# dayne-2stacks/Fingerprint-Matching-Code

Hardware: AMD Instinct MI355X
Metric: graph-match pairs/sec @ n=256 kpts, batch=1024, 1 & 8 GPU (higher is better)
Workload: dtype bf16

## Files before the change

fingerprint-matching-code_amd/csrc/gemm.hip:

```cpp
#include "gemm_phase.h"
#include "gemm_pp.h"
#include <cstdlib>
#include <cstring>

namespace fpm {
int& gemm_bn256_min();
}

extern "C" int fpm_gemm(int dtype, const void* A, long lda, long sA, const int* a_rows, const void* B, long ldb,
                        long sB, int M, int N, int K, int batch, int epi, const float* bias, float* Cf, void* Ct,
                        long ldc, long sC, const int* n1, const int* n2, void* stream) {
    using namespace fpm;
    FPM_CHECK_ARG(dtype == 0 || dtype == 1, "gemm: dtype must be 0 (f32) or 1 (bf16)");
    FPM_CHECK_ARG(M >= 0 && N > 0 && K > 0 && batch >= 0, "gemm: bad sizes M=%d N=%d K=%d", M, N, K);
    FPM_CHECK_ARG(K % (dtype ? 8 : 4) == 0, "gemm: K=%d must be a multiple of %d", K, dtype ? 8 : 4);
    FPM_CHECK_ARG(lda % (dtype ? 8 : 4) == 0 && ldb % (dtype ? 8 : 4) == 0, "gemm: lda/ldb must keep rows 16-B aligned");
    FPM_CHECK_ARG((epi != EPI_AFFINITY && epi != EPI_HALF_AFFINITY) || (n1 && n2),
                  "gemm: affinity epilogues need n1/n2");
    FPM_CHECK_ARG(epi >= EPI_STORE && epi <= EPI_HALF_AFFINITY, "gemm: bad epilogue %d", epi);
    if (M == 0 || batch == 0) return 0;
    GemmParams p = {};
    p.A = A; p.lda = lda; p.sA = sA; p.a_rows = a_rows;
    p.B = B; p.ldb = ldb; p.sB = sB; p.sB_seg = 0;
    p.row_scale = nullptr;
    p.M = M; p.N = N; p.K = K; p.nseg = 1;
    p.tile_info = nullptr; p.group_off = nullptr;
    p.epi = epi; p.bias = bias; p.Cf = Cf; p.Ct = Ct; p.ldc = ldc; p.sC = sC; p.n1 = n1; p.n2 = n2;
    hipStream_t st = (hipStream_t)stream;
    const int mt = (M + G2_BM - 1) / G2_BM;
    const bool epi_ok = epi == EPI_STORE || epi == EPI_RELU || (epi == EPI_AFFINITY && Cf && !Ct);
    const bool big = dtype == 1 && M >= G2_BM && K % G2_BK == 0 && N % 8 == 0 && lda % 8 == 0 && ldb % 8 == 0 &&
                     !(Cf && Ct) && (Cf ? ldc % 4 == 0 : ldc % 8 == 0) && epi_ok &&
                     (long)mt * ((N + 127) / 128) * batch >= 128;
    if (big) {
        const int BN = (N % 256 == 0 && (long)mt * (N / 256) * batch >= gemm_bn256_min()) ? 256 : 128;
        p.remap_mtiles = mt;
        dim3 grid(remap_grid_big(N, BN, mt), 1, batch);
        const bool f32 = Cf != nullptr;
        const bool phase = BN == 256 && use_gemm_phase(K);
#define FPM_BIG(BN_, E_, F_)                                                                            \
    do {                                                                                               \
        if (BN_ == 256 && phase) hipLaunchKernelGGL((gemm_phase_kernel<E_, F_>), grid, dim3(G2_THREADS), 0, st, p); \
        else hipLaunchKernelGGL((gemm_big_kernel<BN_, E_, F_>), grid, dim3(G2_THREADS), 0, st, p);      \
    } while (0)
        if (epi == EPI_AFFINITY) {
            if (BN == 256) FPM_BIG(256, EPI_AFFINITY, true); else FPM_BIG(128, EPI_AFFINITY, true);
        } else if (BN == 256) {
            if (epi == EPI_RELU) { if (f32) FPM_BIG(256, EPI_RELU, true); else FPM_BIG(256, EPI_RELU, false); }
            else { if (f32) FPM_BIG(256, EPI_STORE, true); else FPM_BIG(256, EPI_STORE, false); }
        } else {
            if (epi == EPI_RELU) { if (f32) FPM_BIG(128, EPI_RELU, true); else FPM_BIG(128, EPI_RELU, false); }
            else { if (f32) FPM_BIG(128, EPI_STORE, true); else FPM_BIG(128, EPI_STORE, false); }
        }
#undef FPM_BIG
        return check_launch("fpm_gemm");
    }
    p.remap_mtiles = (M + GBM - 1) / GBM;
    dim3 grid(remap_grid(N, p.remap_mtiles), 1, batch);
    if (dtype == 0) hipLaunchKernelGGL((gemm_kernel<float, false>), grid, dim3(GTHREADS), 0, st, p);
    else hipLaunchKernelGGL((gemm_kernel<bf16_t, false>), grid, dim3(GTHREADS), 0, st, p);
    return check_launch("fpm_gemm");
}

namespace fpm {
int& gemm_pp_flag() {
    static int on = [] {
        const char* e = getenv("FPM_GEMM_PP");
        return e ? atoi(e) : 0;
    }();
    return on;
}

int& gemm_phase_flag() {
    static int on = [] {
        const char* e = getenv("FPM_GEMM_PHASE");
        return e ? atoi(e) : 1;
    }();
    return on;
}

int& gemm_bn256_min() {
    static int v = [] {
        const char* e = getenv("FPM_GEMM_BN256_MIN");
        return e ? atoi(e) : 512;
    }();
    return v;
}
}

extern "C" int fpm_gemm_norm_max(const void* A, long lda, const void* B, long ldb, int M, int N, int K,
                                 const float* bias, const float* res, long ldres, const float* nw, const float* nb,
                                 float eps, int P, float* gmax, void* stream) {
    using namespace fpm;
    FPM_CHECK_ARG(P == G2_BM || 2 * P == G2_BM, "gemm_norm_max: P=%d must be %d or %d (one or two pairs per tile)", P,
                  G2_BM, G2_BM / 2);
    FPM_CHECK_ARG(M >= 0 && M % P == 0 && N > 0 && K > 0 && K % G2_BK == 0, "gemm_norm_max: bad sizes M=%d N=%d K=%d",
                  M, N, K);
    FPM_CHECK_ARG(lda % 8 == 0 && ldb % 8 == 0 && ldres >= N, "gemm_norm_max: bad strides");
    FPM_CHECK_ARG(res && nw && nb && gmax, "gemm_norm_max: null operand");
    if (M == 0) return 0;
    GemmParams p = {};
    p.A = A; p.lda = lda; p.B = B; p.ldb = ldb;
    p.M = M; p.N = N; p.K = K; p.nseg = 1;
    p.epi = EPI_NORM_MAX; p.bias = bias; p.ldc = ldres;
    p.res = res; p.nw = nw; p.nb = nb; p.eps = eps; p.gmax = gmax; p.norm_p = P;
    const int mt = (M + G2_BM - 1) / G2_BM;
    p.remap_mtiles = mt;
    dim3 grid(remap_grid_big(N, 128, mt), 1, 1);
    hipLaunchKernelGGL((gemm_big_kernel<128, EPI_NORM_MAX, true>), grid, dim3(G2_THREADS), 0, (hipStream_t)stream, p);
    return fpm::check_launch("fpm_gemm_norm_max");
}
// ... 77 lines not shown
    float* X1c = ws + (long)B * d;
    if (fpm_gemm(0, w, kw, 0, nullptr, A_w, kw, 0, B, d, kw, 1, EPI_TANH, A_b, coef, nullptr, d, 0, nullptr, nullptr,
                 stream))
        return 1;
    hipLaunchKernelGGL(rows_scale_kernel, dim3((unsigned)((long)B * n1max)), dim3(256), 0, (hipStream_t)stream, X1,
                       ld1, n1max, d, coef, X1c);
    if (check_launch("fpm_affinity_fwd")) return 1;
    return fpm_gemm(0, X1c, d, (long)n1max * d, nullptr, X2, ld2, (long)n2max * ld2, n1max, n2max, d, B,
                    epi == 0 ? EPI_AFFINITY : EPI_HALF_AFFINITY, nullptr, K, nullptr, ldk, (long)n1max * ldk, n2, n1,
                    stream);
}

int& plan_graph_flag();
int& combine_npb_flag();
int& sinkhorn_bwd_reg_flag();
int& sinkhorn_fast_flag();
int& sinkhorn_lform_flag();
int& soft_topk_fast_flag();
int& afau_attn_v_flag();
int& gnn_store_sc1_flag();
int& combine_store_sc1_flag();
int& gemm_store_sc1_flag();
int& combine_lds_kb_flag();
int& gnn_mlp_off_flag();
int& outer_sum_vec_flag();
int& gnn_sweeps_flag();
int& scatter_f32_rows_flag();
int& scatter_batch_flag();
int& afau_head_split_flag();

extern "C" int fpm_set_tuning(const char* key, int value) {
    int* f = nullptr;
    if (key && !strcmp(key, "gemm_phase")) f = &fpm::gemm_phase_flag();
    else if (key && !strcmp(key, "gemm_pp")) f = &fpm::gemm_pp_flag();
    else if (key && !strcmp(key, "plan_graph")) f = &plan_graph_flag();
    else if (key && !strcmp(key, "combine_npb")) f = &combine_npb_flag();
    else if (key && !strcmp(key, "sinkhorn_bwd_reg")) f = &sinkhorn_bwd_reg_flag();
    else if (key && !strcmp(key, "sinkhorn_fast")) f = &sinkhorn_fast_flag();
    else if (key && !strcmp(key, "sinkhorn_lform")) f = &sinkhorn_lform_flag();
    else if (key && !strcmp(key, "topk_fast")) f = &soft_topk_fast_flag();
    else if (key && !strcmp(key, "afau_attn_v")) f = &afau_attn_v_flag();
    else if (key && !strcmp(key, "gnn_store_sc1")) f = &gnn_store_sc1_flag();
    else if (key && !strcmp(key, "combine_store_sc1")) f = &combine_store_sc1_flag();
    else if (key && !strcmp(key, "gemm_store_sc1")) f = &gemm_store_sc1_flag();
    else if (key && !strcmp(key, "combine_lds_kb")) f = &combine_lds_kb_flag();
    else if (key && !strcmp(key, "gnn_mlp_off")) f = &gnn_mlp_off_flag();
    else if (key && !strcmp(key, "outer_sum_vec")) f = &outer_sum_vec_flag();
    else if (key && !strcmp(key, "gnn_sweeps")) f = &gnn_sweeps_flag();
    else if (key && !strcmp(key, "scatter_f32_rows")) f = &scatter_f32_rows_flag();
    else if (key && !strcmp(key, "scatter_batch")) f = &scatter_batch_flag();
    else if (key && !strcmp(key, "afau_head_split")) f = &afau_head_split_flag();
    if (!f) {
        fpm::set_error("fpm_set_tuning: unknown key '%s'", key ? key : "(null)");
        return -1;
    }
    if (f == &gnn_mlp_off_flag() && value != 0) {
        const char* e = getenv("FPM_TIMING_PROBES");
        if (!e || strcmp(e, "1") != 0) {
            fpm::set_error("fpm_set_tuning: '%s' is a timing probe with wrong results; set FPM_TIMING_PROBES=1 "
                           "to allow it", key);
            return -1;
        }
    }
    const int prev = *f;
    *f = value;
    return prev;
}
// ... 156 lines not shown
```

fingerprint-matching-code_amd/csrc/gemm_core.h:

```cpp
#pragma once
#include "fpm_common.h"

namespace fpm {

enum GemmEpi : int {
    EPI_STORE = 0,
    EPI_RELU = 1,
    EPI_TANH = 2,
    EPI_AFFINITY = 3,
    EPI_HALF_AFFINITY = 4,
    EPI_NORM_MAX = 5,
    EPI_NORM_OUT = 6,
};

struct GemmParams {
    const void* A;
    long lda, sA;
    const int* a_rows;
    const void* B;
    long ldb, sB, sB_seg;
    const float* row_scale;
    int M, N, K, nseg;
    const int* tile_info;
    const int* group_off;
    int epi;
    const float* bias;
    float* Cf;
    void* Ct;
    long ldc, sC;
    const int* n1;
    const int* n2;
    int remap_mtiles;
    const float* res;
    const float* nw;
    const float* nb;
    float eps;
    float* gmax;
    long ldt;
    int split;
    int norm_p;
    int store_sc1;
    int remap_cm;
};

constexpr int REMAP_MIN = 32;
inline unsigned remap_grid(int N, int mtiles) {
    long nt = (N + 127) / 128, chunk = 4 * nt;
    long t = nt * mtiles;
    if (mtiles < REMAP_MIN) return (unsigned)t;
    return (unsigned)((t + 8 * chunk - 1) / (8 * chunk) * (8 * chunk));
}
__device__ __forceinline__ int remap_tile(int nt, int mtiles, int cm = 4) {
    if (mtiles < REMAP_MIN) return blockIdx.x;
    const int chunk = cm * nt;
    const int i = blockIdx.x >> 3;
    return ((i / chunk) * 8 + (blockIdx.x & 7)) * chunk + (i % chunk);
}

typedef __bf16 bf16x8_t __attribute__((ext_vector_type(8)));
typedef float f32x4_t __attribute__((ext_vector_type(4)));

template <typename T> struct TileCfg;
template <> struct TileCfg<float> {
    static constexpr int BK = 32;
    static constexpr int EPC = 4;
};
template <> struct TileCfg<bf16_t> {
    static constexpr int BK = 64;
    static constexpr int EPC = 8;
};

constexpr int GBM = 128, GBN = 128, GTHREADS = 256;
constexpr int LDS_ROW_BYTES = 144;
constexpr int LDS_TILE_BYTES = GBM * LDS_ROW_BYTES;

// ... 197 lines not shown
```

fingerprint-matching-code_amd/csrc/gemm_phase.h:

```cpp
#pragma once
#include <type_traits>
#include "gemm_big.h"

namespace fpm {

constexpr int GP_HALF = 128 * 128;
constexpr int GP_SMEM = g2_max(8 * GP_HALF, G2_BM * (2 * 256 + 16));
constexpr int GP_MIN_KTILES = 2;

#define FPM_VMCNT(N) asm volatile("s_waitcnt vmcnt(" #N ")" ::: "memory")

#ifdef GP_PROBE
__device__ unsigned long long* gp_probe_buf;
#define GP_STAMP(k)                                                                                   \
    do {                                                                                              \
        const unsigned long long t_ = __builtin_amdgcn_s_memtime();                                   \
        if (threadIdx.x == 0 && gp_probe_buf)                                                         \
            gp_probe_buf[((long)blockIdx.z * gridDim.x + blockIdx.x) * 8 + (k)] = t_;                   \
    } while (0)
#else
#define GP_STAMP(k)
#endif

#ifndef GP_STAGGER
// ... 263 lines not shown
                for (int fm = 0; fm < 4; ++fm)
#pragma unroll
                    for (int j = 0; j < 4; ++j) {
                        const int r = wr * 64 + fm * 16 + (lane >> 4) * 4 + j;
#pragma unroll
                        for (int fn = 0; fn < 2; ++fn) {
                            const int c = g * 128 + wc * 32 + fn * 16 + (lane & 15);
                            const int n = n0 + c < p.N ? n0 + c : p.N - 1;
                            *(float*)(smem + r * ROW + c * 4) =
                                g2_epi<EPI, HB>(p.bias, acc[h][g][fm][fn][j], row0 + h * 128 + r, n, n1b, n2b);
                        }
                    }
        };
#pragma unroll
        for (int h = 0; h < 2; ++h) {
            if (p.bias) image(h, std::true_type{});
            else image(h, std::false_type{});
            __syncthreads();
#pragma unroll 4
            for (int it = 0; it < 128 * CH / G2_THREADS; ++it) {
                const int idx = it * G2_THREADS + tid;
                const int r = idx / CH, ch = idx % CH;
                const int gr = row0 + h * 128 + r;
                if (gr < row_end && n0 + ch * 4 < p.N) {
                    uint4 v = *(const uint4*)(smem + r * ROW + ch * 16);
                    *(uint4*)(Cf + (long)gr * p.ldc + n0 + ch * 4) = v;
                }
            }
            __syncthreads();
        }
    }
}

#undef FPM_VMCNT

int& gemm_phase_flag();
inline bool use_gemm_phase(int K) { return gemm_phase_flag() != 0 && K / G2_BK >= GP_MIN_KTILES; }

}
```

fingerprint-matching-code_amd/csrc/gemm_pp.h:

```cpp
#pragma once
#include <type_traits>
#include "gemm_big.h"

namespace fpm {

constexpr int PP_BM = 256, PP_BN = 128, PP_BK = 32, PP_THREADS = 256, PP_NST = 3;
constexpr int PP_A_BYTES = PP_BM * PP_BK * 2;
constexpr int PP_B_BYTES = PP_BN * PP_BK * 2;
constexpr int PP_STAGE = PP_A_BYTES + PP_B_BYTES;
constexpr int PP_ROW_OUT = PP_BN * 2 + 16;
constexpr int PP_SMEM = g2_max(PP_NST * PP_STAGE, PP_BM * PP_ROW_OUT);
static_assert(PP_SMEM <= 80 * 1024, "two workgroups per CU need <= 80 KB of LDS each");

inline unsigned pp_grid(int N, int mtiles) { return remap_grid_big(N, PP_BN, mtiles); }

__device__ __forceinline__ int pp_slot(int chunk, int row) {
    return ((0x2130 >> (4 * chunk)) & 3) ^ ((row >> 2) & 3);
}
__device__ __forceinline__ int pp_chunk(int slot, int row) {
    return (0x1320 >> (4 * (slot ^ ((row >> 2) & 3)))) & 3;
}

template <int EPI>
__global__ __launch_bounds__(PP_THREADS, 2) void gemm_pp_kernel(GemmParams p) {
    __shared__ __attribute__((aligned(16))) unsigned char smem[PP_SMEM];
    const int tid = threadIdx.x, lane = tid & 63, wave = tid >> 6;
    const int wr = wave >> 1, wc = wave & 1;
    const int batch = blockIdx.z;

    const int nt = (p.N + PP_BN - 1) / PP_BN;
    const int q = remap_tile(nt, p.remap_mtiles);
    const int mtile = q / nt, ntile = q - mtile * nt;
    if (mtile >= p.remap_mtiles) return;
    int group = 0, row0, row_end;
    if (p.tile_info) {
        group = p.tile_info[2 * mtile];
        if (group < 0) return;
        row0 = p.tile_info[2 * mtile + 1];
        row_end = p.group_off[group + 1];
    } else {
        row0 = mtile * PP_BM;
        row_end = p.M;
    }
    const int n0 = ntile * PP_BN;
    const bf16_t* A = (const bf16_t*)p.A + (long)batch * p.sA;
    const bf16_t* Bg = (const bf16_t*)p.B + (long)batch * p.sB + (long)group * p.sB_seg;

    const bf16_t* asrc[4];
    const bf16_t* bsrc[2];
#pragma unroll
    for (int i = 0; i < 4; ++i) {
        const int r = (wave * 4 + i) * 16 + (lane >> 2);
        int gr = row0 + r;
        gr = gr < row_end ? gr : row0;
        const long arow = p.a_rows ? (long)p.a_rows[gr] : (long)gr;
        asrc[i] = A + arow * p.lda + pp_chunk(lane & 3, r) * 8;
    }
#pragma unroll
    for (int i = 0; i < 2; ++i) {
        const int r = (wave * 2 + i) * 16 + (lane >> 2);
        const int n = n0 + r < p.N ? n0 + r : p.N - 1;
        bsrc[i] = Bg + (long)n * p.ldb + pp_chunk(lane & 3, r) * 8;
    }
    auto issue = [&](int stage, int kt) {
        unsigned char* As = smem + stage * PP_STAGE;
        unsigned char* Bs = As + PP_A_BYTES;
        const int k0 = kt * PP_BK;
#pragma unroll
        for (int i = 0; i < 4; ++i)
            __builtin_amdgcn_global_load_lds((gbl_ptr_t)(asrc[i] + k0), (lds_ptr_t)(As + (wave * 4 + i) * 1024), 16,
                                             0, 0);
#pragma unroll
        for (int i = 0; i < 2; ++i)
            __builtin_amdgcn_global_load_lds((gbl_ptr_t)(bsrc[i] + k0), (lds_ptr_t)(Bs + (wave * 2 + i) * 1024), 16,
                                             0, 0);
    };

    const int so = pp_slot(lane >> 4, lane & 15) * 16;
    const int a_off = (wr * 64 + (lane & 15)) * 64 + so;
    const int b_off = (wc * 64 + (lane & 15)) * 64 + so;

    f32x4_t acc[2][4][4];
#pragma unroll
    for (int h = 0; h < 2; ++h)
#pragma unroll
        for (int i = 0; i < 4; ++i)
#pragma unroll
            for (int j = 0; j < 4; ++j) acc[h][i][j] = f32x4_t{0.f, 0.f, 0.f, 0.f};

    auto compute = [&](int stage) __attribute__((always_inline)) {
        const unsigned char* As = smem + stage * PP_STAGE;
        const unsigned char* Bs = As + PP_A_BYTES;
        bf16x8_t a[2][4], b[4];
#pragma unroll
        for (int f = 0; f < 4; ++f) b[f] = *(const bf16x8_t*)(Bs + b_off + f * 1024);
#pragma unroll
        for (int h = 0; h < 2; ++h)
#pragma unroll
            for (int f = 0; f < 4; ++f) a[h][f] = *(const bf16x8_t*)(As + a_off + h * 8192 + f * 1024);
#pragma unroll
        for (int h = 0; h < 2; ++h)
#pragma unroll
            for (int fm = 0; fm < 4; ++fm)
#pragma unroll
                for (int fn = 0; fn < 4; ++fn)
                    acc[h][fm][fn] = __builtin_amdgcn_mfma_f32_16x16x32_bf16(a[h][fm], b[fn], acc[h][fm][fn], 0, 0, 0);
    };

    const int ktiles = p.K / PP_BK;
    issue(0, 0);
    if (ktiles > 1) issue(1, 1);
    for (int kt = 0; kt < ktiles; ++kt) {
        if (kt + 1 < ktiles) asm volatile("s_waitcnt vmcnt(6)" ::: "memory");
        else asm volatile("s_waitcnt vmcnt(0)" ::: "memory");
        __builtin_amdgcn_s_barrier();
        if (kt + 2 < ktiles) issue((kt + 2) % PP_NST, kt + 2);
        compute(kt % PP_NST);
    }
    __syncthreads();

    int n1b = 0, n2b = 0;
    if (EPI == EPI_AFFINITY) { n1b = p.n1[batch]; n2b = p.n2[batch]; }
    constexpr int ROW = PP_ROW_OUT;
    const int lr = wr * 64 + (lane >> 4) * 4, lc = wc * 64 + (lane & 15);
    auto image = [&](auto hb) __attribute__((always_inline)) {
        constexpr bool HB = decltype(hb)::value;
#pragma unroll
        for (int h = 0; h < 2; ++h) {
            int wo = (h * 128 + lr) * ROW + lc * 2;
            asm volatile("" : "+v"(wo));
            unsigned char* wb = smem + wo;
#pragma unroll
            for (int fm = 0; fm < 4; ++fm)
#pragma unroll
                for (int j = 0; j < 4; j += 2) {
                    const int r = h * 128 + lr + fm * 16 + j;
#pragma unroll
                    for (int fn = 0; fn < 4; ++fn) {
                        const int c = lc + fn * 16;
                        const int n = n0 + c < p.N ? n0 + c : p.N - 1;
                        const uint32_t pk =
                            f2bf2(g2_epi<EPI, HB>(p.bias, acc[h][fm][fn][j], row0 + r, n, n1b, n2b),
                                  g2_epi<EPI, HB>(p.bias, acc[h][fm][fn][j + 1], row0 + r + 1, n, n1b, n2b));
                        const int off = (fm * 16 + j) * ROW + fn * 32;
                        *(bf16_t*)(wb + off) = (bf16_t)pk;
                        *(bf16_t*)(wb + off + ROW) = (bf16_t)(pk >> 16);
                    }
                }
        }
    };
    if (p.bias) image(std::true_type{});
    else image(std::false_type{});
    __syncthreads();
    bf16_t* Ct = (bf16_t*)p.Ct + (long)batch * p.sC;
    constexpr int CH = PP_BN / 8;
    if (p.store_sc1) {
        typedef unsigned int u32x4_t __attribute__((ext_vector_type(4)));
        const __amdgpu_buffer_rsrc_t rc = __builtin_amdgcn_make_buffer_rsrc(
            (void*)(Ct + (long)row0 * p.ldc + n0), (short)0, (int)(PP_BM * p.ldc * 2), 0x00020000);
#pragma unroll 4
        for (int it = 0; it < PP_BM * CH / PP_THREADS; ++it) {
            const int idx = it * PP_THREADS + tid;
            const int r = idx / CH, ch = idx % CH;
            if (row0 + r < row_end && n0 + ch * 8 < p.N) {
                const uint4 v = *(const uint4*)(smem + r * ROW + ch * 16);
                const u32x4_t pk = {v.x, v.y, v.z, v.w};
                __builtin_amdgcn_raw_buffer_store_b128(pk, rc, (int)((r * p.ldc + ch * 8) * 2), 0, 16);
            }
        }
    } else {
#pragma unroll 4
        for (int it = 0; it < PP_BM * CH / PP_THREADS; ++it) {
            const int idx = it * PP_THREADS + tid;
            const int r = idx / CH, ch = idx % CH;
            if (row0 + r < row_end && n0 + ch * 8 < p.N) {
                const uint4 v = *(const uint4*)(smem + r * ROW + ch * 16);
                *(uint4*)(Ct + (long)(row0 + r) * p.ldc + n0 + ch * 8) = v;
            }
        }
    }
}

int& gemm_pp_flag();
inline bool use_gemm_pp(int K) { return gemm_pp_flag() != 0 && K % 64 == 0 && K >= PP_BK; }

}
```

fingerprint-matching-code_amd/csrc/spline.hip:

```cpp
#include "gemm_phase.h"
#include "gemm_pp.h"

#include <vector>

namespace {

struct ProfRec {
    hipEvent_t a, b;
    int slot;
};
bool g_prof_on = false;
std::vector<ProfRec> g_prof;
int* g_prof_rows = nullptr;
constexpr int PROF_MAX = 4096;

constexpr int NCELL = 26;

struct PlanLayout {
    long mask, indeg, dslot, basis_e, grp_e, blk_cnt, cell_off, rowid, arows, tile_info, tile_info2, dst_ptr, csr_e,
        nbr_local, rows4, basis4, total;
    long nblk, max_rows, max_tiles, max_tiles2;
};

__host__ __device__ inline long al(long x) { return (x + 255) & ~255L; }

__host__ __device__ inline long plan_max_rows(long E, long num_nodes) {
    long a = 4 * E, b = 25 * num_nodes;
    return (a < b ? a : b) + num_nodes;
}

__host__ __device__ PlanLayout plan_layout(long E, long num_nodes) {
    PlanLayout L;
    L.nblk = (num_nodes + 255) / 256;
    L.max_rows = plan_max_rows(E, num_nodes);
// ... 1093 lines not shown
                                   void* stream) {
    return fpm_spline_conv_fwd_argmax(dtype, x_op, plan_ws, E, num_nodes, nmax, nvalid, W, bias, y_ws, y_ws_bytes, mode,
                                      xres, cscale, out_f, out_t, nullptr, stream);
}

extern "C" int fpm_spline_conv_fwd_argmax(int dtype, const void* x_op, const void* plan_ws, long E, long num_nodes,
                                          int nmax, const int* nvalid, const void* W, const float* bias, void* y_ws,
                                          long y_ws_bytes, int mode, const float* xres, const float* cscale,
                                          float* out_f, void* out_t, int* argmax, void* stream) {
    using namespace fpm;
    FPM_CHECK_ARG(dtype == 0 || dtype == 1, "spline_conv: bad dtype");
    FPM_CHECK_ARG(mode >= 0 && mode <= 5 && (!(mode & 1) || xres), "spline_conv: mode %d: bit 0 (residual) needs xres, "
                  "mode >> 1 must be 0, 1 or 2", mode);
    FPM_CHECK_ARG(!(mode >> 1) || (dtype == 1 && out_t && !argmax),
                  "spline_conv: split operand rows (mode >> 1) need bf16 out_t (inference forward)");
    FPM_CHECK_ARG(y_ws_bytes >= fpm_spline_y_bytes(dtype, E, num_nodes), "spline_conv: y workspace too small");
    PlanLayout L = plan_layout(E, num_nodes);
    const char* w = (const char*)plan_ws;
    hipStream_t st = (hipStream_t)stream;
    const int D = 768;
    {
        GemmParams p = {};
        p.A = x_op; p.lda = D; p.a_rows = (const int*)(w + L.arows);
        p.B = W; p.ldb = D; p.sB_seg = (long)D * D;
        p.M = (int)L.max_rows; p.N = D; p.K = D; p.nseg = 1;
        p.tile_info = (const int*)(w + L.tile_info);
        p.group_off = (const int*)(w + L.cell_off);
        p.epi = EPI_STORE; p.ldc = D;
        if (dtype == 0) p.Cf = (float*)y_ws;
        else p.Ct = y_ws;
        p.store_sc1 = gemm_store_sc1_flag();
        p.remap_mtiles = (int)(dtype == 0 ? L.max_tiles : L.max_tiles2);
        if (dtype == 1) p.tile_info = (const int*)(w + L.tile_info2);
        const bool pp = dtype == 1 && use_gemm_pp(D);
        dim3 grid(dtype == 0 ? remap_grid(D, p.remap_mtiles) : pp ? pp_grid(D, p.remap_mtiles)
                                                                  : remap_grid256(D, p.remap_mtiles), 1, 1);
        ProfRec rec = {nullptr, nullptr, (int)g_prof.size()};
        if (g_prof_on && !g_prof_rows) (void)hipMalloc(&g_prof_rows, PROF_MAX * sizeof(int));
        if (g_prof_on && g_prof_rows && rec.slot < PROF_MAX) {
            (void)hipMemcpyAsync(g_prof_rows + rec.slot, w + L.cell_off + NCELL * sizeof(int), sizeof(int),
                                 hipMemcpyDeviceToDevice, st);
            (void)hipEventCreate(&rec.a);
            (void)hipEventCreate(&rec.b);
            (void)hipEventRecord(rec.a, st);
        }
        if (dtype == 0) hipLaunchKernelGGL((gemm_kernel<float, false>), grid, dim3(GTHREADS), 0, st, p);
        else if (pp) hipLaunchKernelGGL((gemm_pp_kernel<EPI_STORE>), grid, dim3(PP_THREADS), 0, st, p);
        else if (use_gemm_phase(D)) hipLaunchKernelGGL((gemm_phase_kernel<EPI_STORE, false>), grid, dim3(G2_THREADS), 0, st, p);
        else hipLaunchKernelGGL((gemm_big_kernel<256, EPI_STORE, false>), grid, dim3(G2_THREADS), 0, st, p);
        if (g_prof_on && g_prof_rows && rec.slot < PROF_MAX) {
            (void)hipEventRecord(rec.b, st);
            g_prof.push_back(rec);
        }
    }
    {
        const long graphs = (num_nodes + nmax - 1) / nmax;
        const int npb = combine_npb_flag();
#define FPM_COMB(T_, N_)                                                                                         \
    do {                                                                                                         \
        const dim3 cg((unsigned)(((graphs + 7) / 8) * 8 * ((nmax + N_ - 1) / N_)));                              \
        const size_t lds = (size_t)combine_lds_kb_flag() * 1024;                                                 \
        if (combine_store_sc1_flag() && !(mode >> 1))                                                            \
            hipLaunchKernelGGL((combine_kernel<T_, N_, false, 16>), cg, dim3(64 * N_), lds, st, (const T_*)y_ws, \
                               (const int*)(w + L.cell_off), bias, (const int*)(w + L.dst_ptr),                 \
                               (const int4*)(w + L.rows4), (const float4*)(w + L.basis4), num_nodes, nmax,       \
                               nvalid, mode, xres, cscale, out_f, (T_*)out_t, nullptr);                          \
        else                                                                                                     \
            hipLaunchKernelGGL((combine_kernel<T_, N_>), cg, dim3(64 * N_), lds, st, (const T_*)y_ws,            \
                               (const int*)(w + L.cell_off), bias, (const int*)(w + L.dst_ptr),                 \
                               (const int4*)(w + L.rows4), (const float4*)(w + L.basis4), num_nodes, nmax,       \
                               nvalid, mode, xres, cscale, out_f, (T_*)out_t, nullptr);                          \
    } while (0)
        if (argmax) {
#define FPM_COMBA(T_)                                                                                            \
    hipLaunchKernelGGL((combine_kernel<T_, 4, true>), dim3((unsigned)(((graphs + 7) / 8) * 8 * ((nmax + 3) / 4))), \
                       dim3(256), 0, st, (const T_*)y_ws, (const int*)(w + L.cell_off), bias,                    \
                       (const int*)(w + L.dst_ptr), (const int4*)(w + L.rows4), (const float4*)(w + L.basis4),   \
                       num_nodes, nmax, nvalid, mode, xres, cscale, out_f, (T_*)out_t, argmax)
            if (dtype == 0) FPM_COMBA(float); else FPM_COMBA(bf16_t);
#undef FPM_COMBA
// ... 374 lines not shown
```

Before: 32220.

## Add strip-walking bf16 GEMM kernel that processes two M-tiles per workgroup

New measurement: 32760, median of 6. 1.7% higher.

```diff
diff --git a/fingerprint-matching-code_amd/csrc/gemm.hip b/fingerprint-matching-code_amd/csrc/gemm.hip
--- a/fingerprint-matching-code_amd/csrc/gemm.hip
+++ b/fingerprint-matching-code_amd/csrc/gemm.hip
@@ -1,11 +1,11 @@
 #include "gemm_phase.h"
-#include "gemm_pp.h"
 #include <cstdlib>
 #include <cstring>
 
 namespace fpm {
 int& gemm_bn256_min();
 }
+int& gemm_store_sc1_flag();
 
 extern "C" int fpm_gemm(int dtype, const void* A, long lda, long sA, const int* a_rows, const void* B, long ldb,
                         long sB, int M, int N, int K, int batch, int epi, const float* bias, float* Cf, void* Ct,
@@ -47,7 +47,13 @@
             if (BN == 256) FPM_BIG(256, EPI_AFFINITY, true); else FPM_BIG(128, EPI_AFFINITY, true);
         } else if (BN == 256) {
             if (epi == EPI_RELU) { if (f32) FPM_BIG(256, EPI_RELU, true); else FPM_BIG(256, EPI_RELU, false); }
-            else { if (f32) FPM_BIG(256, EPI_STORE, true); else FPM_BIG(256, EPI_STORE, false); }
+            else if (f32) FPM_BIG(256, EPI_STORE, true);
+            else {
+                const int S = phase ? gemm_walk_strip(p) : 0;
+                p.store_sc1 = gemm_store_sc1_flag();
+                if (S != 0) gemm_walk_launch(p, S, batch, st);
+                else FPM_BIG(256, EPI_STORE, false);
+            }
         } else {
             if (epi == EPI_RELU) { if (f32) FPM_BIG(128, EPI_RELU, true); else FPM_BIG(128, EPI_RELU, false); }
             else { if (f32) FPM_BIG(128, EPI_STORE, true); else FPM_BIG(128, EPI_STORE, false); }
@@ -63,20 +69,31 @@
 }
 
 namespace fpm {
-int& gemm_pp_flag() {
-    static int on = [] {
-        const char* e = getenv("FPM_GEMM_PP");
-        return e ? atoi(e) : 0;
-    }();
-    return on;
-}
-
 int& gemm_phase_flag() {
     static int on = [] {
         const char* e = getenv("FPM_GEMM_PHASE");
         return e ? atoi(e) : 1;
     }();
     return on;
+}
+
+int& gemm_walk_flag() {
+    static int v = [] {
+        const char* e = getenv("FPM_GEMM_WALK");
+        return e ? atoi(e) : GW_AUTO;
+    }();
+    return v;
+}
+
+int gemm_cu_count() {
+    static int cus = [] {
+        int dev = 0, n = 0;
+        if (hipGetDevice(&dev) != hipSuccess ||
+            hipDeviceGetAttribute(&n, hipDeviceAttributeMultiprocessorCount, dev) != hipSuccess || n <= 0)
+            n = 256;
+        return n;
+    }();
+    return cus;
 }
 
 int& gemm_bn256_min() {
@@ -220,7 +237,8 @@
 extern "C" int fpm_set_tuning(const char* key, int value) {
     int* f = nullptr;
     if (key && !strcmp(key, "gemm_phase")) f = &fpm::gemm_phase_flag();
-    else if (key && !strcmp(key, "gemm_pp")) f = &fpm::gemm_pp_flag();
+    else if (key && !strcmp(key, "gemm_walk")) f = &fpm::gemm_walk_flag();
+    else if (key && !strcmp(key, "gemm_bn256_min")) f = &fpm::gemm_bn256_min();
     else if (key && !strcmp(key, "plan_graph")) f = &plan_graph_flag();
     else if (key && !strcmp(key, "combine_npb")) f = &combine_npb_flag();
     else if (key && !strcmp(key, "sinkhorn_bwd_reg")) f = &sinkhorn_bwd_reg_flag();
diff --git a/fingerprint-matching-code_amd/csrc/gemm_core.h b/fingerprint-matching-code_amd/csrc/gemm_core.h
--- a/fingerprint-matching-code_amd/csrc/gemm_core.h
+++ b/fingerprint-matching-code_amd/csrc/gemm_core.h
@@ -41,6 +41,9 @@
     int norm_p;
     int store_sc1;
     int remap_cm;
+    int walk;
+    const int* tile_count;
+    int walk_cus;
 };
 
 constexpr int REMAP_MIN = 32;
diff --git a/fingerprint-matching-code_amd/csrc/gemm_phase.h b/fingerprint-matching-code_amd/csrc/gemm_phase.h
--- a/fingerprint-matching-code_amd/csrc/gemm_phase.h
+++ b/fingerprint-matching-code_amd/csrc/gemm_phase.h
@@ -319,9 +319,334 @@
     }
 }
 
+constexpr int GW_SMEM = 8 * GP_HALF;
+constexpr int GW_MAX_S = 2;
+
+__host__ __device__ inline int gemm_walk_rule(int tiles, int wgs, int cus) {
+    const long r1 = ((long)tiles * wgs + cus - 1) / cus, r2 = ((long)((tiles + 1) / 2) * wgs + cus - 1) / cus;
+    return 2 * r2 * 7 <= r1 * 8 ? 2 : 1;
+}
+
+#ifdef GP_PROBE
+#define GW_STAMP(k) do { if (ti == 0) GP_STAMP(k); } while (0)
+#else
+#define GW_STAMP(k)
+#endif
+
+template <bool SC1>
+__global__ __launch_bounds__(G2_THREADS, 1) void gemm_walk_kernel(GemmParams p) {
+    constexpr int BN = 256;
+    __shared__ __attribute__((aligned(16))) unsigned char smem[GW_SMEM];
+    const int tid = threadIdx.x, lane = tid & 63, wave = tid >> 6;
+    const int wr = wave >> 2, wc = wave & 3;
+    const int batch = blockIdx.z;
+
+    const int nt = p.N / BN;
+    int mtiles = p.remap_mtiles;
+    if (p.tile_count) mtiles = *p.tile_count < mtiles ? *p.tile_count : mtiles;
+    const int S = p.walk > 0 ? p.walk : gemm_walk_rule(mtiles, nt * (int)gridDim.z, p.walk_cus);
+    const int strips = (mtiles + S - 1) / S;
+    const int i = blockIdx.x >> 3;
+    const int strip = (i / nt) * 8 + (blockIdx.x & 7), ntile = i % nt;
+    if (strip >= strips) return;
+    int t_row0[GW_MAX_S], t_rend[GW_MAX_S], t_grp[GW_MAX_S];
+    unsigned ok = 0;
+#pragma unroll
+    for (int j = 0; j < GW_MAX_S; ++j) {
+        const int mt = strip * S + j;
+        t_row0[j] = 0; t_rend[j] = 0; t_grp[j] = 0;
+        if (j < S && mt < mtiles) {
+            if (p.tile_info) {
+                const int g = p.tile_info[2 * mt];
+                if (g >= 0) {
+                    t_grp[j] = g;
+                    t_row0[j] = p.tile_info[2 * mt + 1];
+                    t_rend[j] = p.group_off[g + 1];
+                    ok |= 1u << j;
+                }
+            } else {
+                t_row0[j] = mt * G2_BM;
+                t_rend[j] = p.M;
+                ok |= 1u << j;
+            }
+        }
+    }
+    if (!ok) return;
+    constexpr int m_end = GW_MAX_S;
+    auto next_valid = [&](int j) __attribute__((always_inline)) {
+        const unsigned r = j < GW_MAX_S ? ok >> j : 0u;
+        return r ? j + __builtin_ctz(r) : GW_MAX_S;
+    };
+    auto pick = [&](const int (&t)[GW_MAX_S], int j) __attribute__((always_inline)) {
+        return j == 0 ? t[0] : t[1];
+    };
+    int m = next_valid(0);
+
+    const int n0 = ntile * BN;
+    const bf16_t* A = (const bf16_t*)p.A + (long)batch * p.sA;
+    const unsigned char* Bb = (const unsigned char*)((const bf16_t*)p.B + (long)batch * p.sB);
+    bf16_t* Ct = (bf16_t*)p.Ct + (long)batch * p.sC;
+
+    auto tile_at = [&](int j, int& row0, int& row_end, const unsigned char*& bg) __attribute__((always_inline)) {
+        row0 = pick(t_row0, j);
+        row_end = pick(t_rend, j);
+        bg = Bb + (long)pick(t_grp, j) * p.sB_seg * 2;
+    };
+    auto a_rows_of = [&](int row0, int row_end, int (&ar)[2][2]) __attribute__((always_inline)) {
+#pragma unroll
+        for (int i = 0; i < 2; ++i)
+#pragma unroll
+            for (int h = 0; h < 2; ++h) {
+                int gr = row0 + h * 128 + (wave * 2 + i) * 8 + (lane >> 3);
+                gr = gr < row_end ? gr : row0;
+                ar[h][i] = p.a_rows ? p.a_rows[gr] : gr;
+            }
+    };
+    const uint32_t kc16 = (uint32_t)(((lane & 7) ^ (lane >> 4)) * 16);
+    uint32_t b_off[2];
+#pragma unroll
+    for (int i = 0; i < 2; ++i)
+        b_off[i] = (uint32_t)((n0 + (wave * 2 + i) * 8 + (lane >> 3)) * (uint32_t)p.ldb * 2) + (kc16 ^ (i * 64));
+    const uint32_t lda2 = (uint32_t)p.lda * 2, bhalf = 128 * (uint32_t)p.ldb * 2;
+    const unsigned char* Ab = (const unsigned char*)A;
+
+    int row0, row_end, row0n = 0, row_endn = 0;
+    const unsigned char *bg, *bgn = nullptr;
+    int ar[2][2], arn[2][2];
+
+    auto issue = [&](int slot, int buf, const int (&rows)[2][2], const unsigned char* bgrp, int k0) __attribute__((always_inline)) {
+        unsigned char* dst = smem + (buf * 4 + slot) * GP_HALF + wave * 2048;
+        if (slot < 2) {
+            const unsigned char* ab = Ab + 2 * k0;
+#pragma unroll
+            for (int i = 0; i < 2; ++i)
+                __builtin_amdgcn_global_load_lds(
+                    (gbl_ptr_t)(ab + ((uint64_t)(uint32_t)rows[slot][i] * lda2 + (kc16 ^ (i * 64)))),
+                    (lds_ptr_t)(dst + i * 1024), 16, 0, 0);
+        } else {
+            const unsigned char* b = bgrp + 2 * k0 + (slot - 2) * bhalf;
+            __builtin_amdgcn_global_load_lds((gbl_ptr_t)(b + b_off[0]), (lds_ptr_t)dst, 16, 0, 0);
+            __builtin_amdgcn_global_load_lds((gbl_ptr_t)(b + b_off[1]), (lds_ptr_t)(dst + 1024), 16, 0, 0);
+        }
+    };
+
+    const int xr = (lane >> 1) & 7;
+    const int a_off = (wr * 64 + (lane & 15)) * 128;
+    const int b_offl = (wc * 32 + (lane & 15)) * 128;
+    const int s0 = ((lane >> 4) ^ xr) * 16, s1 = ((4 + (lane >> 4)) ^ xr) * 16;
+
+    f32x4_t acc[2][2][4][2];
+    auto zero_acc = [&]() __attribute__((always_inline)) {
+#pragma unroll
+        for (int h = 0; h < 2; ++h)
+#pragma unroll
+            for (int g = 0; g < 2; ++g)
+#pragma unroll
+                for (int i = 0; i < 4; ++i)
+#pragma unroll
+                    for (int j = 0; j < 2; ++j) acc[h][g][i][j] = f32x4_t{0.f, 0.f, 0.f, 0.f};
+    };
+    bf16x8_t a[2][4], b0[2][2], b1[2][2];
+
+    auto read_a = [&](int u, int h) __attribute__((always_inline)) {
+        const unsigned char* base = smem + ((u & 1) * 4 + h) * GP_HALF + a_off;
+#pragma unroll
+        for (int f = 0; f < 4; ++f) {
+            a[0][f] = *(const bf16x8_t*)(base + f * 2048 + s0);
+            a[1][f] = *(const bf16x8_t*)(base + f * 2048 + s1);
+        }
+    };
+    auto read_b = [&](int u, int g, bf16x8_t (&bb)[2][2]) __attribute__((always_inline)) {
+        const unsigned char* base = smem + ((u & 1) * 4 + 2 + g) * GP_HALF + b_offl;
+#pragma unroll
+        for (int f = 0; f < 2; ++f) {
+            bb[0][f] = *(const bf16x8_t*)(base + f * 2048 + s0);
+            bb[1][f] = *(const bf16x8_t*)(base + f * 2048 + s1);
+        }
+    };
+    auto mfma = [&](f32x4_t (&c)[4][2], bf16x8_t (&bb)[2][2]) __attribute__((always_inline)) {
+        __builtin_amdgcn_s_barrier();
+        asm volatile("s_waitcnt lgkmcnt(0)" ::: "memory");
+        if (GP_PRIO) __builtin_amdgcn_s_setprio(1);
+#pragma unroll
+        for (int kk = 0; kk < 2; ++kk)
+#pragma unroll
+            for (int fm = 0; fm < 4; ++fm)
+#pragma unroll
+                for (int fn = 0; fn < 2; ++fn)
+                    c[fm][fn] = __builtin_amdgcn_mfma_f32_16x16x32_bf16(bb[kk][fn], a[kk][fm], c[fm][fn], 0, 0, 0);
+        if (GP_PRIO) __builtin_amdgcn_s_setprio(0);
+        __builtin_amdgcn_s_barrier();
+    };
+    constexpr int NONE = 0, CUR = 1, NEXT = 2;
+    auto wait = [&](int v) __attribute__((always_inline)) {
+        if (v == 6) FPM_VMCNT(6);
+        else if (v == 4) FPM_VMCNT(4);
+        else if (v == 2) FPM_VMCNT(2);
+        else if (v == 0) FPM_VMCNT(0);
+    };
+    auto iss = [&](int mode, int slot, int buf, int k0) __attribute__((always_inline)) {
+        if (mode == CUR) issue(slot, buf, ar, bg, k0);
+        else if (mode == NEXT) issue(slot, buf, arn, bgn, 0);
+    };
+    auto ktile = [&](int u, int k1, int VM0, int VM1, int VM2, int VM3, int M01, int M23) __attribute__((always_inline)) {
+        asm volatile("" : "+s"(k1));
+        wait(VM0);
+        iss(M01, 3, (u + 1) & 1, k1);
+        read_a(u, 0);
+        read_b(u, 0, b0);
+        mfma(acc[0][0], b0);
+        wait(VM1);
+        iss(M01, 1, (u + 1) & 1, k1);
+        read_b(u, 1, b1);
+        mfma(acc[0][1], b1);
+        wait(VM2);
+        iss(M23, 0, u & 1, k1 + G2_BK);
+        read_a(u, 1);
+        mfma(acc[1][1], b1);
+        wait(VM3);
+        iss(M23, 2, u & 1, k1 + G2_BK);
+        mfma(acc[1][0], b0);
+    };
+
+    auto epilogue = [&](int buf, auto hb) __attribute__((always_inline)) {
+        constexpr bool HB = decltype(hb)::value;
+        unsigned char* img = smem + buf * (4 * GP_HALF);
+        int tid_ = tid;
+        asm volatile("" : "+v"(tid_));
+        const int lane = tid_ & 63, wr = tid_ >> 8, wc = (tid_ >> 6) & 3;
+        int wbase[2];
+#pragma unroll
+        for (int fn = 0; fn < 2; ++fn)
+            wbase[fn] = (wr * 64 + (lane & 15)) * 512 + (((wc * 4 + fn * 2 + (lane >> 5)) ^ (lane & 7)) << 4) +
+                        ((lane >> 4) & 1) * 8;
+        const int rb_r = tid_ >> 5, rb_c = tid_ & 31;
+        const int rbase = rb_r * 512 + ((rb_c ^ (rb_r & 7)) << 4);
+        const int cl = n0 + wc * 32 + 4 * (lane >> 4);
+#pragma unroll
+        for (int h = 0; h < 2; ++h) {
+#pragma unroll
+            for (int g = 0; g < 2; ++g)
+#pragma unroll
+                for (int fm = 0; fm < 4; ++fm)
+#pragma unroll
+                    for (int fn = 0; fn < 2; ++fn) {
+                        const f32x4_t v = acc[h][g][fm][fn];
+                        const int n = cl + g * 128 + fn * 16;
+                        uint2 o;
+                        o.x = f2bf2(g2_epi<EPI_STORE, HB>(p.bias, v[0], 0, n, 0, 0),
+                                    g2_epi<EPI_STORE, HB>(p.bias, v[1], 0, n + 1, 0, 0));
+                        o.y = f2bf2(g2_epi<EPI_STORE, HB>(p.bias, v[2], 0, n + 2, 0, 0),
+                                    g2_epi<EPI_STORE, HB>(p.bias, v[3], 0, n + 3, 0, 0));
+                        *(uint2*)(img + wbase[fn] + fm * 8192 + g * 256) = o;
+                    }
+            asm volatile("s_waitcnt lgkmcnt(0)" ::: "memory");
+            __builtin_amdgcn_s_barrier();
+            const int rbeg = row0 + h * 128 + rb_r;
+            if constexpr (SC1) {
+                typedef unsigned int u32x4_t __attribute__((ext_vector_type(4)));
+                const __amdgpu_buffer_rsrc_t rc = __builtin_amdgcn_make_buffer_rsrc(
+                    (void*)(Ct + (long)row0 * p.ldc + n0), (short)0, (int)(G2_BM * p.ldc * 2), 0x00020000);
+#pragma unroll
+                for (int it = 0; it < 8; ++it) {
+                    const uint4 v = *(const uint4*)(img + rbase + it * 8192);
+                    if (rbeg + it * 16 < row_end) {
+                        const u32x4_t pk = {v.x, v.y, v.z, v.w};
+                        __builtin_amdgcn_raw_buffer_store_b128(
+                            pk, rc, (int)(((h * 128 + rb_r + it * 16) * p.ldc + rb_c * 8) * 2), 0, 16);
+                    }
+                }
+            } else {
+#pragma unroll
+                for (int it = 0; it < 8; ++it) {
+                    const uint4 v = *(const uint4*)(img + rbase + it * 8192);
+                    if (rbeg + it * 16 < row_end) *(uint4*)(Ct + (long)(rbeg + it * 16) * p.ldc + n0 + rb_c * 8) = v;
+                }
+            }
+            asm volatile("s_waitcnt lgkmcnt(0)" ::: "memory");
+            __builtin_amdgcn_s_barrier();
+        }
+    };
+
+    const int T = p.K / G2_BK;
+    tile_at(m, row0, row_end, bg);
+    a_rows_of(row0, row_end, ar);
+    int mn = next_valid(m + 1);
+    if (mn < m_end) {
+        tile_at(mn, row0n, row_endn, bgn);
+        a_rows_of(row0n, row_endn, arn);
+    }
+    issue(0, 0, ar, bg, 0);
+    issue(2, 0, ar, bg, 0);
+    issue(3, 0, ar, bg, 0);
+    issue(1, 0, ar, bg, 0);
+    issue(0, 1, ar, bg, G2_BK);
+    issue(2, 1, ar, bg, G2_BK);
+    zero_acc();
+    FPM_VMCNT(8);
+    __builtin_amdgcn_s_barrier();
+
+    int u = 0;
+#ifdef GP_PROBE
+    int ti = 0;
+#endif
+    for (;;) {
+        const bool has_next = mn < m_end;
+        GW_STAMP(0);
+        if (GP_STAGGER && wr == 1) __builtin_amdgcn_s_barrier();
+        int k1 = G2_BK;
+        for (int t = 0; t < T - 2; ++t, ++u, k1 += G2_BK) ktile(u, k1, 6, 6, 6, 6, CUR, CUR);
+        ktile(u, k1, 6, 6, 6, has_next ? 6 : 4, CUR, has_next ? NEXT : NONE);
+        GW_STAMP(1);
+        ktile(u + 1, 0, has_next ? 6 : 2, has_next ? 6 : 0, -1, -1, has_next ? NEXT : NONE, NONE);
+        ++u;
+        if (GP_STAGGER && wr == 0) __builtin_amdgcn_s_barrier();
+        GW_STAMP(2);
+        if (p.bias) epilogue(u & 1, std::true_type{});
+        else epilogue(u & 1, std::false_type{});
+        GW_STAMP(3);
+        if (!has_next) break;
+        m = mn; mn = m_end;
+        row0 = row0n; row_end = row_endn; bg = bgn;
+#pragma unroll
+        for (int h = 0; h < 2; ++h)
+#pragma unroll
+            for (int i = 0; i < 2; ++i) ar[h][i] = arn[h][i];
+        issue(0, u & 1, ar, bg, G2_BK);
+        issue(2, u & 1, ar, bg, G2_BK);
+        FPM_VMCNT(4);
+        zero_acc();
+        __builtin_amdgcn_s_barrier();
+        GW_STAMP(4);
+        ++u;
+#ifdef GP_PROBE
+        ++ti;
+#endif
+    }
+}
+
 #undef FPM_VMCNT
 
 int& gemm_phase_flag();
 inline bool use_gemm_phase(int K) { return gemm_phase_flag() != 0 && K / G2_BK >= GP_MIN_KTILES; }
 
+constexpr int GW_AUTO = 8;
+int& gemm_walk_flag();
+int gemm_cu_count();
+inline int gemm_walk_strip(const GemmParams& p) {
+    const int f = gemm_walk_flag();
+    if (f <= 1 || !use_gemm_phase(p.K) || p.N % 256 != 0 || !p.Ct || p.Cf || p.epi != EPI_STORE) return 0;
+    if ((long)p.N * p.ldb * 2 >= (1L << 31) || (long)G2_BM * p.ldc * 2 >= (1L << 31) || p.lda >= (1L << 31)) return 0;
+    return f < GW_AUTO ? 2 : GW_AUTO;
 }
+inline void gemm_walk_launch(GemmParams p, int S, int batch, hipStream_t st) {
+    const long nt = p.N / 256;
+    p.walk_cus = gemm_cu_count();
+    p.walk = S == 2 || p.remap_mtiles * nt * batch >= 8L * gemm_cu_count() ? 2 : 0;
+    const int strips = p.walk ? (p.remap_mtiles + 1) / 2 : p.remap_mtiles;
+    const dim3 grid((unsigned)((strips + 7) / 8 * 8 * nt), 1, batch);
+    if (p.store_sc1) hipLaunchKernelGGL((gemm_walk_kernel<true>), grid, dim3(G2_THREADS), 0, st, p);
+    else hipLaunchKernelGGL((gemm_walk_kernel<false>), grid, dim3(G2_THREADS), 0, st, p);
+}
+
+}
diff --git a/fingerprint-matching-code_amd/csrc/gemm_pp.h b/fingerprint-matching-code_amd/csrc/gemm_pp.h
--- a/fingerprint-matching-code_amd/csrc/gemm_pp.h
+++ /dev/null
@@ -1,187 +0,0 @@
-#pragma once
-#include <type_traits>
-#include "gemm_big.h"
-
-namespace fpm {
-
-constexpr int PP_BM = 256, PP_BN = 128, PP_BK = 32, PP_THREADS = 256, PP_NST = 3;
-constexpr int PP_A_BYTES = PP_BM * PP_BK * 2;
-constexpr int PP_B_BYTES = PP_BN * PP_BK * 2;
-constexpr int PP_STAGE = PP_A_BYTES + PP_B_BYTES;
-constexpr int PP_ROW_OUT = PP_BN * 2 + 16;
-constexpr int PP_SMEM = g2_max(PP_NST * PP_STAGE, PP_BM * PP_ROW_OUT);
-static_assert(PP_SMEM <= 80 * 1024, "two workgroups per CU need <= 80 KB of LDS each");
-
-inline unsigned pp_grid(int N, int mtiles) { return remap_grid_big(N, PP_BN, mtiles); }
-
-__device__ __forceinline__ int pp_slot(int chunk, int row) {
-    return ((0x2130 >> (4 * chunk)) & 3) ^ ((row >> 2) & 3);
-}
-__device__ __forceinline__ int pp_chunk(int slot, int row) {
-    return (0x1320 >> (4 * (slot ^ ((row >> 2) & 3)))) & 3;
-}
-
-template <int EPI>
-__global__ __launch_bounds__(PP_THREADS, 2) void gemm_pp_kernel(GemmParams p) {
-    __shared__ __attribute__((aligned(16))) unsigned char smem[PP_SMEM];
-    const int tid = threadIdx.x, lane = tid & 63, wave = tid >> 6;
-    const int wr = wave >> 1, wc = wave & 1;
-    const int batch = blockIdx.z;
-
-    const int nt = (p.N + PP_BN - 1) / PP_BN;
-    const int q = remap_tile(nt, p.remap_mtiles);
-    const int mtile = q / nt, ntile = q - mtile * nt;
-    if (mtile >= p.remap_mtiles) return;
-    int group = 0, row0, row_end;
-    if (p.tile_info) {
-        group = p.tile_info[2 * mtile];
-        if (group < 0) return;
-        row0 = p.tile_info[2 * mtile + 1];
-        row_end = p.group_off[group + 1];
-    } else {
-        row0 = mtile * PP_BM;
-        row_end = p.M;
-    }
-    const int n0 = ntile * PP_BN;
-    const bf16_t* A = (const bf16_t*)p.A + (long)batch * p.sA;
-    const bf16_t* Bg = (const bf16_t*)p.B + (long)batch * p.sB + (long)group * p.sB_seg;
-
-    const bf16_t* asrc[4];
-    const bf16_t* bsrc[2];
-#pragma unroll
-    for (int i = 0; i < 4; ++i) {
-        const int r = (wave * 4 + i) * 16 + (lane >> 2);
-        int gr = row0 + r;
-        gr = gr < row_end ? gr : row0;
-        const long arow = p.a_rows ? (long)p.a_rows[gr] : (long)gr;
-        asrc[i] = A + arow * p.lda + pp_chunk(lane & 3, r) * 8;
-    }
-#pragma unroll
-    for (int i = 0; i < 2; ++i) {
-        const int r = (wave * 2 + i) * 16 + (lane >> 2);
-        const int n = n0 + r < p.N ? n0 + r : p.N - 1;
-        bsrc[i] = Bg + (long)n * p.ldb + pp_chunk(lane & 3, r) * 8;
-    }
-    auto issue = [&](int stage, int kt) {
-        unsigned char* As = smem + stage * PP_STAGE;
-        unsigned char* Bs = As + PP_A_BYTES;
-        const int k0 = kt * PP_BK;
-#pragma unroll
-        for (int i = 0; i < 4; ++i)
-            __builtin_amdgcn_global_load_lds((gbl_ptr_t)(asrc[i] + k0), (lds_ptr_t)(As + (wave * 4 + i) * 1024), 16,
-                                             0, 0);
-#pragma unroll
-        for (int i = 0; i < 2; ++i)
-            __builtin_amdgcn_global_load_lds((gbl_ptr_t)(bsrc[i] + k0), (lds_ptr_t)(Bs + (wave * 2 + i) * 1024), 16,
-                                             0, 0);
-    };
-
-    const int so = pp_slot(lane >> 4, lane & 15) * 16;
-    const int a_off = (wr * 64 + (lane & 15)) * 64 + so;
-    const int b_off = (wc * 64 + (lane & 15)) * 64 + so;
-
-    f32x4_t acc[2][4][4];
-#pragma unroll
-    for (int h = 0; h < 2; ++h)
-#pragma unroll
-        for (int i = 0; i < 4; ++i)
-#pragma unroll
-            for (int j = 0; j < 4; ++j) acc[h][i][j] = f32x4_t{0.f, 0.f, 0.f, 0.f};
-
-    auto compute = [&](int stage) __attribute__((always_inline)) {
-        const unsigned char* As = smem + stage * PP_STAGE;
-        const unsigned char* Bs = As + PP_A_BYTES;
-        bf16x8_t a[2][4], b[4];
-#pragma unroll
-        for (int f = 0; f < 4; ++f) b[f] = *(const bf16x8_t*)(Bs + b_off + f * 1024);
-#pragma unroll
-        for (int h = 0; h < 2; ++h)
-#pragma unroll
-            for (int f = 0; f < 4; ++f) a[h][f] = *(const bf16x8_t*)(As + a_off + h * 8192 + f * 1024);
-#pragma unroll
-        for (int h = 0; h < 2; ++h)
-#pragma unroll
-            for (int fm = 0; fm < 4; ++fm)
-#pragma unroll
-                for (int fn = 0; fn < 4; ++fn)
-                    acc[h][fm][fn] = __builtin_amdgcn_mfma_f32_16x16x32_bf16(a[h][fm], b[fn], acc[h][fm][fn], 0, 0, 0);
-    };
-
-    const int ktiles = p.K / PP_BK;
-    issue(0, 0);
-    if (ktiles > 1) issue(1, 1);
-    for (int kt = 0; kt < ktiles; ++kt) {
-        if (kt + 1 < ktiles) asm volatile("s_waitcnt vmcnt(6)" ::: "memory");
-        else asm volatile("s_waitcnt vmcnt(0)" ::: "memory");
-        __builtin_amdgcn_s_barrier();
-        if (kt + 2 < ktiles) issue((kt + 2) % PP_NST, kt + 2);
-        compute(kt % PP_NST);
-    }
-    __syncthreads();
-
-    int n1b = 0, n2b = 0;
-    if (EPI == EPI_AFFINITY) { n1b = p.n1[batch]; n2b = p.n2[batch]; }
-    constexpr int ROW = PP_ROW_OUT;
-    const int lr = wr * 64 + (lane >> 4) * 4, lc = wc * 64 + (lane & 15);
-    auto image = [&](auto hb) __attribute__((always_inline)) {
-        constexpr bool HB = decltype(hb)::value;
-#pragma unroll
-        for (int h = 0; h < 2; ++h) {
-            int wo = (h * 128 + lr) * ROW + lc * 2;
-            asm volatile("" : "+v"(wo));
-            unsigned char* wb = smem + wo;
-#pragma unroll
-            for (int fm = 0; fm < 4; ++fm)
-#pragma unroll
-                for (int j = 0; j < 4; j += 2) {
-                    const int r = h * 128 + lr + fm * 16 + j;
-#pragma unroll
-                    for (int fn = 0; fn < 4; ++fn) {
-                        const int c = lc + fn * 16;
-                        const int n = n0 + c < p.N ? n0 + c : p.N - 1;
-                        const uint32_t pk =
-                            f2bf2(g2_epi<EPI, HB>(p.bias, acc[h][fm][fn][j], row0 + r, n, n1b, n2b),
-                                  g2_epi<EPI, HB>(p.bias, acc[h][fm][fn][j + 1], row0 + r + 1, n, n1b, n2b));
-                        const int off = (fm * 16 + j) * ROW + fn * 32;
-                        *(bf16_t*)(wb + off) = (bf16_t)pk;
-                        *(bf16_t*)(wb + off + ROW) = (bf16_t)(pk >> 16);
-                    }
-                }
-        }
-    };
-    if (p.bias) image(std::true_type{});
-    else image(std::false_type{});
-    __syncthreads();
-    bf16_t* Ct = (bf16_t*)p.Ct + (long)batch * p.sC;
-    constexpr int CH = PP_BN / 8;
-    if (p.store_sc1) {
-        typedef unsigned int u32x4_t __attribute__((ext_vector_type(4)));
-        const __amdgpu_buffer_rsrc_t rc = __builtin_amdgcn_make_buffer_rsrc(
-            (void*)(Ct + (long)row0 * p.ldc + n0), (short)0, (int)(PP_BM * p.ldc * 2), 0x00020000);
-#pragma unroll 4
-        for (int it = 0; it < PP_BM * CH / PP_THREADS; ++it) {
-            const int idx = it * PP_THREADS + tid;
-            const int r = idx / CH, ch = idx % CH;
-            if (row0 + r < row_end && n0 + ch * 8 < p.N) {
-                const uint4 v = *(const uint4*)(smem + r * ROW + ch * 16);
-                const u32x4_t pk = {v.x, v.y, v.z, v.w};
-                __builtin_amdgcn_raw_buffer_store_b128(pk, rc, (int)((r * p.ldc + ch * 8) * 2), 0, 16);
-            }
-        }
-    } else {
-#pragma unroll 4
-        for (int it = 0; it < PP_BM * CH / PP_THREADS; ++it) {
-            const int idx = it * PP_THREADS + tid;
-            const int r = idx / CH, ch = idx % CH;
-            if (row0 + r < row_end && n0 + ch * 8 < p.N) {
-                const uint4 v = *(const uint4*)(smem + r * ROW + ch * 16);
-                *(uint4*)(Ct + (long)(row0 + r) * p.ldc + n0 + ch * 8) = v;
-            }
-        }
-    }
-}
-
-int& gemm_pp_flag();
-inline bool use_gemm_pp(int K) { return gemm_pp_flag() != 0 && K % 64 == 0 && K >= PP_BK; }
-
-}
diff --git a/fingerprint-matching-code_amd/csrc/spline.hip b/fingerprint-matching-code_amd/csrc/spline.hip
--- a/fingerprint-matching-code_amd/csrc/spline.hip
+++ b/fingerprint-matching-code_amd/csrc/spline.hip
@@ -1,5 +1,4 @@
 #include "gemm_phase.h"
-#include "gemm_pp.h"
 
 #include <vector>
 
@@ -1159,9 +1158,9 @@
         p.store_sc1 = gemm_store_sc1_flag();
         p.remap_mtiles = (int)(dtype == 0 ? L.max_tiles : L.max_tiles2);
         if (dtype == 1) p.tile_info = (const int*)(w + L.tile_info2);
-        const bool pp = dtype == 1 && use_gemm_pp(D);
-        dim3 grid(dtype == 0 ? remap_grid(D, p.remap_mtiles) : pp ? pp_grid(D, p.remap_mtiles)
-                                                                  : remap_grid256(D, p.remap_mtiles), 1, 1);
+        const int walk = dtype == 1 ? gemm_walk_strip(p) : 0;
+        p.tile_count = (const int*)(w + L.cell_off) + NCELL + 2;
+        dim3 grid(dtype == 0 ? remap_grid(D, p.remap_mtiles) : remap_grid256(D, p.remap_mtiles), 1, 1);
         ProfRec rec = {nullptr, nullptr, (int)g_prof.size()};
         if (g_prof_on && !g_prof_rows) (void)hipMalloc(&g_prof_rows, PROF_MAX * sizeof(int));
         if (g_prof_on && g_prof_rows && rec.slot < PROF_MAX) {
@@ -1172,7 +1171,7 @@
             (void)hipEventRecord(rec.a, st);
         }
         if (dtype == 0) hipLaunchKernelGGL((gemm_kernel<float, false>), grid, dim3(GTHREADS), 0, st, p);
-        else if (pp) hipLaunchKernelGGL((gemm_pp_kernel<EPI_STORE>), grid, dim3(PP_THREADS), 0, st, p);
+        else if (walk != 0) gemm_walk_launch(p, walk, 1, st);
         else if (use_gemm_phase(D)) hipLaunchKernelGGL((gemm_phase_kernel<EPI_STORE, false>), grid, dim3(G2_THREADS), 0, st, p);
         else hipLaunchKernelGGL((gemm_big_kernel<256, EPI_STORE, false>), grid, dim3(G2_THREADS), 0, st, p);
         if (g_prof_on && g_prof_rows && rec.slot < PROF_MAX) {
```
